# Lalwaniamisha789/Implementation-of-Neural-LDPC-Decoders-with-Degree-Specific-Weight-Sharing-and-RCQ-Quantization

Hardware: AMD Instinct MI355X
Metric: decoded codewords/sec at fixed iters; achieved HBM GB/s vs peak (higher is better)
Workload: dtype f32; 1 GPU; (1998,1512) IRA code, BasicMinSumDecoder factor=0.7, fp32, 10 iterations, batch 65536/GPU, SNR 2.0 dB, fixed-iteration flooding decode; graph=ira_1998_1512, n=1998, m=486, edges=6587, batch_per_gpu=65536, global_batch=65536, parallelism=dp1, collective=none

## Files before the change

### implementation-of-neural-ldpc-decoders-with-degree-specific-weight-sharing-and-rcq-quantization_amd/_native.py

```python

from __future__ import annotations

import ctypes as C
import os
import subprocess
import threading
from typing import Optional

import numpy as np

_HERE = os.path.dirname(os.path.abspath(__file__))
LIB_NAME = "libldpc_hip.so"
LIB_PATH = os.environ.get("LDPC_HIP_LIB") or os.path.join(_HERE, LIB_NAME)
CSRC = os.path.join(_HERE, "csrc")
HEADER = os.path.join(os.path.dirname(_HERE), "include", "ldpc_hip.h")
DEBUG_HEADER = os.path.join(os.path.dirname(_HERE), "include", "ldpc_hip_debug.h")

LDPC_F32, LDPC_F64 = 0, 1
C2V_NMS, C2V_RCQ, C2V_OMS = 0, 1, 2
MODE_AUTO, MODE_STREAM, MODE_RESIDENT, MODE_SWEEPS, MODE_GATHER, MODE_PAIR = 0, 1, 2, 3, 4, 5
SCHED_FLOODING, SCHED_LAYERED_REF, SCHED_LAYERED = 0, 1, 2

HIPCC_FLAGS = ["--offload-arch=gfx950", "-O3", "-std=c++17", "-fPIC", "-shared",
               "-ffp-contract=off",
# ... 67 lines not shown
                ("n_beta_slots", C.c_int32), ("beta", C.c_void_p), ("beta_slot", C.c_void_p),
                ("n_alpha_slots", C.c_int32), ("alpha", C.c_void_p), ("alpha_slot", C.c_void_p),
                ("n_levels", C.c_int32), ("n_quantizers", C.c_int32), ("thresholds", C.c_void_p),
                ("q_of_iter", C.c_void_p),
                ("n_oms_alpha_slots", C.c_int32), ("oms_alpha", C.c_void_p), ("oms_alpha_slot", C.c_void_p),
                ("schedule", C.c_int32)]


PRODUCT_EXPORTS = ("ldpc_graph_create", "ldpc_graph_destroy", "ldpc_graph_info", "ldpc_decoder_create",
                   "ldpc_decoder_set_mode", "ldpc_decoder_info",
                   "ldpc_decoder_set_weights", "ldpc_decoder_destroy", "ldpc_decoder_workspace_bytes",
                   "ldpc_decode", "ldpc_decode_capped", "ldpc_last_error", "ldpc_abi_version", "ldpc_source_hash",
                   "ldpc_train_saved_bytes", "ldpc_train_workspace_bytes", "ldpc_decode_saving", "ldpc_backward",
                   "ldpc_train_joint_workspace_bytes", "ldpc_train_joint")
DEBUG_EXPORTS = ("ldpc_debug_sweep", "ldpc_debug_workspace_layout", "ldpc_debug_resident_c2v", "ldpc_debug_key4",
                 "ldpc_debug_compact_layout", "ldpc_debug_compact_checks", "ldpc_debug_compact_banks")
EXPORTS = PRODUCT_EXPORTS + DEBUG_EXPORTS

_lib = None
_lock = threading.Lock()


def load():
    global _lib
    if _lib is not None:
        return _lib
    with _lock:
        if _lib is not None:
            return _lib
        if not os.path.exists(LIB_PATH):
            raise NativeEngineError(
# ... 32 lines not shown
        lib.ldpc_decode_capped.argtypes = [vp, vp, i64, i32, i32, vp, vp, vp, vp, vp, vp, C.c_size_t, vp]
        lib.ldpc_debug_sweep.restype = C.c_int
        lib.ldpc_debug_sweep.argtypes = [vp, i64, i32, i32, vp, C.c_size_t, vp]
        lib.ldpc_debug_workspace_layout.restype = C.c_int
        lib.ldpc_debug_workspace_layout.argtypes = [vp, i64, i32, vp]
        lib.ldpc_debug_key4.restype = C.c_int
        lib.ldpc_debug_key4.argtypes = [vp, i64, C.c_float, vp, vp, vp, vp]
        lib.ldpc_debug_resident_c2v.restype = C.c_int
        lib.ldpc_debug_resident_c2v.argtypes = [vp, vp, i64, i32, i32, vp, vp, vp, vp]
        lib.ldpc_debug_compact_layout.restype = C.c_int
        lib.ldpc_debug_compact_layout.argtypes = [vp, i32, i32, i32, vp, vp, vp, vp, vp]
        lib.ldpc_debug_compact_banks.restype = C.c_int
        lib.ldpc_debug_compact_banks.argtypes = [vp, i32, i32, i32, vp, vp, vp, vp, vp, vp, vp, vp, vp]
        lib.ldpc_debug_compact_checks.restype = C.c_int
        lib.ldpc_debug_compact_checks.argtypes = [vp, i32, i32, i32, vp, vp, vp]
        lib.ldpc_train_saved_bytes.restype = C.c_size_t
        lib.ldpc_train_saved_bytes.argtypes = [vp, i64]
        lib.ldpc_train_workspace_bytes.restype = C.c_size_t
        lib.ldpc_train_workspace_bytes.argtypes = [vp, i64]
        lib.ldpc_decode_saving.restype = C.c_int
        lib.ldpc_decode_saving.argtypes = [vp, vp, i64, i32, vp, vp, vp, vp, vp, C.c_size_t, vp, C.c_size_t, vp]
        lib.ldpc_backward.restype = C.c_int
        lib.ldpc_backward.argtypes = [vp, vp, C.c_size_t, vp, i64, vp, vp, vp, vp, vp, vp, vp, C.c_size_t, vp]
        lib.ldpc_train_joint_workspace_bytes.restype = C.c_size_t
        lib.ldpc_train_joint_workspace_bytes.argtypes = [vp, i64]
        lib.ldpc_train_joint.restype = C.c_int
        lib.ldpc_train_joint.argtypes = [vp, vp, vp, i64, vp, vp, vp, vp, vp, vp, vp, vp, vp, C.c_size_t, vp]
        lib.ldpc_last_error.restype = C.c_char_p
        lib.ldpc_last_error.argtypes = []
        lib.ldpc_abi_version.restype = C.c_int
# ... 22 lines not shown
```

### implementation-of-neural-ldpc-decoders-with-degree-specific-weight-sharing-and-rcq-quantization_amd/csrc/ldpc_hip.hip

```cpp
#include "ldpc_kernels.hip"
#include "ldpc_resident.hip"
#include "ldpc_train.hip"
#include "ldpc_layered.hip"

#include <algorithm>
#include <climits>
#include <mutex>
#include <set>
#include <cmath>
#include <cstdarg>
#include <cstdio>
#include <cstdlib>
#include <cstring>
#include <exception>
#include <new>
#include <vector>

#include "../../include/ldpc_hip.h"
#include "../../include/ldpc_hip_debug.h"

using namespace ldpc;

namespace {

// ... 1282 lines not shown

void cpt_layout(const ldpc_graph *g, const std::vector<ResVCheck> &vc, long long S, CptLayout &L)
{
    const int n = g->n;
    std::vector<int> dv(n);
    for (int j = 0; j < n; ++j) dv[j] = g->h_var_ptr[j + 1] - g->h_var_ptr[j];
    if (!cpt_assign(dv, L) || (long long)L.var_at.size() > S) {
        L.var_at.resize(n);
        for (int j = 0; j < n; ++j) L.var_at[j] = j;
        std::stable_sort(L.var_at.begin(), L.var_at.end(), [&](int a, int b) { return dv[a] > dv[b]; });
    }
    cpt_place_banks(g, vc, L);
    cpt_cells(dv, L);
}

int resident_layout(ldpc_decoder *d, const ldpc_decoder_desc *desc, const std::vector<ResVCheck> &sorted, int mstride,
                    long long S, int G, ResidentPlan &pl, const CptLayout *cl)
{
    const ldpc_graph *g = d->g;
    std::vector<ResVCheck> placed;
    if (cl)
        for (int c : cl->check_at) placed.push_back(sorted[c]);
    const std::vector<ResVCheck> &vc = cl ? placed : sorted;
    const int n = g->n, m = (int)vc.size();
    const bool any_split = m != g->m;
    int max_sub = 0;
    for (const ResVCheck &v : vc) max_sub = std::max(max_sub, v.dc);
    std::vector<int> perm_v(n), pos_v(n);
    for (int j = 0; j < n; ++j) perm_v[j] = j;
    auto dv_of = [&](int j) { return g->h_var_ptr[j + 1] - g->h_var_ptr[j]; };
    std::stable_sort(perm_v.begin(), perm_v.end(), [&](int a, int b) { return dv_of(a) > dv_of(b); });
    std::vector<int> slot_of_edge(g->E);
    for (int p = 0; p < m; ++p)
        for (int t = 0; t < vc[p].dc; ++t) slot_of_edge[vc[p].e0 + t] = t * mstride + p;
    if (cl) {
        perm_v = cl->var_at;
        slot_of_edge = cl->slot_of_edge;
    } else {
        std::vector<std::vector<int>> vs(n);
        for (int j = 0; j < n; ++j)
            for (int k = 0; k < dv_of(j); ++k) vs[j].push_back(slot_of_edge[g->h_csc[g->h_var_ptr[j] + k]]);
        optimise_lane_order(perm_v, vs, G);
    }
    const int n_pos = (int)perm_v.size();
    const int n_ent = cl ? (n_pos + 63) / 64 * 64 : n;
    for (int q = 0; q < n_pos; ++q)
        if (perm_v[q] >= 0) pos_v[perm_v[q]] = q;

    std::vector<uint8_t> dc_s(m), gsz(m);
    std::vector<uint16_t> cvar((size_t)S, 0), bslot((size_t)S, 0), oaslot((size_t)S, 0), bslot_c(m, 0), inv(n);
    std::vector<uint32_t> vmeta(n_ent, 0u);
    std::vector<uint2> vslot_lo(n_ent, make_uint2(0, kResHole)), vslot_hi(std::max(n_ent, 1), make_uint2(0, 0));
    int n_hi = 0;
    std::vector<uint32_t> edge_of_slot((size_t)S, 0xffffffffu);
    bool per_check = true;
    for (int p = 0; p < m; ++p) {
        const ResVCheck &v = vc[p];
        const int first = g->h_check_ptr[v.check];
        dc_s[p] = (uint8_t)v.dc;
        gsz[p] = (uint8_t)v.gs;
        for (int t = 0; t < v.dc; ++t) {
            const int e = v.e0 + t, slot = slot_of_edge[e];
            edge_of_slot[slot] = (uint32_t)e;
            cvar[slot] = (uint16_t)pos_v[g->h_var_idx[e]];
            bslot[slot] = (uint16_t)desc->beta_slot[e];
            if (desc->beta_slot[e] != desc->beta_slot[first]) per_check = false;
            if (d->form == LDPC_C2V_OMS && desc->oms_alpha) oaslot[slot] = (uint16_t)desc->oms_alpha_slot[e];
        }
        bslot_c[p] = v.dc ? (uint16_t)desc->beta_slot[first] : 0;
    }
    for (int q = 0; q < n_pos; ++q) {
        if (perm_v[q] < 0) continue;
        const int j = perm_v[q], s0 = g->h_var_ptr[j], dv = dv_of(j);
        vmeta[q] = (uint32_t)dv | ((uint32_t)desc->alpha_slot[j] << 8);
        inv[j] = (uint16_t)q;
        uint32_t off[8] = {0, 0, 0, 0, 0, 0, 0, 0};
        for (int k = 0; k < dv; ++k) off[k] = (uint32_t)slot_of_edge[g->h_csc[s0 + k]] * G * 4;
        vslot_lo[q] = make_uint2(off[0] | (off[1] << 16), off[2] | (off[3] << 16));
        vslot_hi[q] = make_uint2(off[4] | (off[5] << 16), off[6] | (off[7] << 16));
        if (dv > 4) n_hi = q + 1;
    }
    pl = ResidentPlan{};
    pl.n = n; pl.m = m; pl.S = (int)S; pl.max_dc = max_sub; pl.max_dv = g->max_dv; pl.mstride = mstride; pl.E = g->E;
    pl.any_split = any_split ? 1 : 0;
    pl.n_hi = n_hi;
    pl.n_pos = n_pos;
    if (cl) {
        std::copy(cl->cell, cl->cell + kCptWaves, pl.vcell);
        cpt_check_words(vc, per_check && (d->form == LDPC_C2V_NMS || (d->form == LDPC_C2V_RCQ && d->rcq_zero0)),
                        pl.ccell);
    }
    pl.par_words = is_pow2(mstride) ? m : 0;
    pl.par_shift = G == 2 ? 3 : 2;
    int rc = plan_upload(d, &pl.dc_s, dc_s);
    if (!rc && any_split) rc = plan_upload(d, &pl.gsz, gsz);
    if (!rc) rc = plan_upload(d, &pl.cvar, cvar);
    if (!rc) rc = plan_upload(d, &pl.bslot, bslot);
    if (!rc && per_check) rc = plan_upload(d, &pl.bslot_c, bslot_c);
    if (!rc && d->form == LDPC_C2V_OMS && desc->oms_alpha) rc = plan_upload(d, &pl.oaslot, oaslot);
    if (!rc) rc = plan_upload(d, &pl.vmeta, vmeta);
    if (!rc) rc = plan_upload(d, &pl.vslot_lo, vslot_lo);
    vslot_hi.resize((size_t)std::max(n_hi, 1));
    if (!rc) rc = plan_upload(d, &pl.vslot_hi, vslot_hi);
    if (!rc) rc = plan_upload(d, &pl.inv_perm_v, inv);
    if (!rc) rc = plan_upload(d, &pl.edge_of_slot, edge_of_slot);
    return rc;
}

int allow_full_lds(const void *kfn, int device)
{
    static std::mutex mu;
    static std::set<std::pair<const void *, int>> done;
    std::lock_guard<std::mutex> lk(mu);
    if (done.count({kfn, device})) return LDPC_OK;
    HIP_TRY(hipFuncSetAttribute(kfn, hipFuncAttributeMaxDynamicSharedMemorySize, (int)kLdsBytes));
    done.insert({kfn, device});
    return LDPC_OK;
// ... 1098 lines not shown
    emit(L->slot_of_edge, L->check_at, L->banks, slot_of_edge, pos_of_check, model);
    emit(L->base_slot_of_edge, L->base_check_at, L->base_banks, base_slot_of_edge, base_pos_of_check, base_model);
    if (geometry) { geometry[0] = kResCptStride; geometry[1] = (int32_t)Sc; }
    return LDPC_OK;
}

int ldpc_debug_compact_banks(const ldpc_decoder *d, int32_t n, int32_t m, int32_t E, const int32_t *check_ptr,
                             const int32_t *var_idx, int32_t *slot_of_edge, int32_t *pos_of_check, int32_t model[4],
                             int32_t *base_slot_of_edge, int32_t *base_pos_of_check, int32_t base_model[4],
                             int32_t geometry[2])
{
    LDPC_NOTHROW(compact_banks_impl(d, n, m, E, check_ptr, var_idx, slot_of_edge, pos_of_check, model, base_slot_of_edge,
                                    base_pos_of_check, base_model, geometry))
}

int ldpc_debug_resident_c2v(const ldpc_decoder *d, const void *llr, int64_t batch, int32_t early_stop,
                            int32_t max_iterations, void *posterior, int32_t *iterations, void *c2v_out, void *stream)
{
    if (!d || !llr || !posterior || !c2v_out || batch <= 0) return fail(LDPC_ERR_ARG, "bad argument");
    if (!use_resident(d)) return fail(LDPC_ERR_ARG, "the decoder is not on the LDS-resident engine");
    if (d->g->n == 0) return LDPC_OK;
    IterCap cap(max_iterations > 0 ? max_iterations : INT_MAX);
    return decode_resident(d, llr, batch, early_stop, nullptr, posterior, iterations, nullptr, nullptr, c2v_out, stream);
}

int ldpc_debug_sweep(const ldpc_decoder *d, int64_t batch, int32_t which, int32_t iter, void *workspace,
                     size_t workspace_bytes, void *stream)
{
    if (!d || !workspace || batch <= 0) return fail(LDPC_ERR_ARG, "bad argument");
    if (iter < 0 || iter >= d->T) return fail(LDPC_ERR_ARG, "iter outside [0, T)");
// ... 35 lines not shown
```

### implementation-of-neural-ldpc-decoders-with-degree-specific-weight-sharing-and-rcq-quantization_amd/csrc/ldpc_resident.hip

```cpp
#pragma once

#include "ldpc_kernels.hip"

namespace ldpc {

struct ResidentPlan {
    int n, m, S, max_dc, max_dv;
    int mstride;
    const uint8_t *dc_s;
    const uint8_t *gsz;
    int any_split;
    int par_words;
    int par_shift;
    const uint16_t *cvar;
    const uint16_t *bslot;
    const uint16_t *bslot_c;
    const uint16_t *oaslot;
    const uint32_t *vmeta;
    const uint2 *vslot_lo;
    const uint2 *vslot_hi;
    int n_hi;
    const uint16_t *inv_perm_v;
    int n_pos;
    unsigned vcell[8];
// ... 490 lines not shown
                const float r = d > 0.0f ? d : 0.0f;
                const float val = r - oa;
                o.x[g] = nonzero ? __uint_as_float(__float_as_uint(val) ^ sflip) : 0.0f;
            } else {
                const float w = __uint_as_float(__float_as_uint(b * raw) ^ sflip);
                const float rec = res_quant_rec<NL>(__builtin_fabsf(w), th, thr, n_levels);
                o.x[g] = flip_sign<float>(rec, (w < 0.0f) ? 1u : 0u);
            }
        }
        lds_store<P>(addr, o);
        slot += sstride;
    }
    }
}

template <int G, int FORM, bool BPC, int NL, int MS, typename T, bool SPLIT, bool CPT = false>
__device__ __forceinline__ void res_check_phase(const ResidentPlan &pl, unsigned char *smem,
                                                const T *__restrict__ beta_row,
                                                const T *__restrict__ oa_row,
                                                const float *__restrict__ thr, int n_levels, bool rcq_zero0,
                                                int dc_pre, T b_pre, int tid, int nt, unsigned cw = 0)
{
    float th[8];
    if (FORM == FORM_RCQ) {
#pragma unroll
        for (int q = 0; q < 8; ++q) th[q] = (q < n_levels) ? thr[q] : __builtin_nanf("");
    }
    if constexpr (CPT && BPC && (FORM == FORM_NMS || FORM == FORM_RCQ)) {
        static_assert(G == 2 && !SPLIT && std::is_same<T, float>::value, "compact: fp32 codeword pairs, whole checks");
        asm volatile("" : "+s"(cw));
// ... 37 lines not shown
    const unsigned off[8] = {slo.x, slo.y, slo.z, slo.w, shi.x, shi.y, shi.z, shi.w};
    P x[DV > 0 ? DV : 1];
#pragma unroll
    for (int k = 0; k < DV; ++k) x[k] = lds_load<P>(off[k]);
    P l = lreg ? *lreg : L[q];
    if constexpr (MODE == 0 || MODE == 2 || MODE == 4 || MODE == 6) {
        P out[DV > 0 ? DV : 1];
        auto v2c = [&](T llr, T sum) { return (MODE & 2) ? llr + sum : llr + a * sum; };
        unsigned byte = 0;
#pragma unroll
        for (int g = 0; g < G; ++g) {
            T xs[DV > 0 ? DV : 1];
#pragma unroll
            for (int k = 0; k < DV; ++k) xs[k] = x[k].x[g];
            if constexpr ((MODE & 4) != 0) byte |= ((l.x[g] + sum_ct<DV, -1, ORD, T>(xs)) < (T)0 ? 1u : 0u) << g;
            if constexpr (DV >= 1) out[0].x[g] = v2c(l.x[g], sum_ct<DV - 1, 0, ORD, T>(xs));
            if constexpr (DV >= 2) out[1].x[g] = v2c(l.x[g], sum_ct<DV - 1, 1, ORD, T>(xs));
            if constexpr (DV >= 3) out[2].x[g] = v2c(l.x[g], sum_ct<DV - 1, 2, ORD, T>(xs));
            if constexpr (DV >= 4) out[3].x[g] = v2c(l.x[g], sum_ct<DV - 1, 3, ORD, T>(xs));
            if constexpr (DV >= 5) out[4].x[g] = v2c(l.x[g], sum_ct<DV - 1, 4, ORD, T>(xs));
            if constexpr (DV >= 6) out[5].x[g] = v2c(l.x[g], sum_ct<DV - 1, 5, ORD, T>(xs));
            if constexpr (DV >= 7) out[6].x[g] = v2c(l.x[g], sum_ct<DV - 1, 6, ORD, T>(xs));
            if constexpr (DV >= 8) out[7].x[g] = v2c(l.x[g], sum_ct<DV - 1, 7, ORD, T>(xs));
        }
#pragma unroll
        for (int k = 0; k < DV; ++k) lds_store<P>(off[k], out[k]);
        if constexpr ((MODE & 4) != 0) {
            bits_s[q] = (uint8_t)byte;
            if (ps.par_off) {
#pragma unroll
                for (int k = 0; k < DV; ++k) lds_atomic_xor(ps.par_off + (((off[k] >> ps.shift) & ps.mask) << 2), byte);
// ... 21 lines not shown
                for (int k = 0; k < DV; ++k) lds_atomic_xor(ps.par_off + (((off[k] >> ps.shift) & ps.mask) << 2), byte);
            }
        }
        if (store) {
            if constexpr (MODE == 9) *lreg = l;
            else L[q] = l;
        }
    }
}

__device__ __forceinline__ uint4 plan_unpack(const uint2 &p)
{
    return make_uint4(p.x & 0xffffu, p.x >> 16, p.y & 0xffffu, p.y >> 16);
}

template <int G, int MODE, typename T, int DMAX = 8>
__device__ __forceinline__ void res_var_dispatch(unsigned char *smem, T *__restrict__ llr_s,
                                                 uint8_t *__restrict__ bits_s, int q, int dv, const uint4 &slo,
                                                 const uint4 &shi, T a, unsigned emask, const ParScatter &ps,
                                                 Pack<T, G> *lreg = nullptr)
{
#define LDPC_RV(D) \
    case D: if constexpr (D <= DMAX) res_var_body<G, D, MODE, T>(smem, llr_s, bits_s, q, slo, shi, a, emask, ps, lreg); break;
    switch (dv) {
        LDPC_RV(0) LDPC_RV(1) LDPC_RV(2) LDPC_RV(3) LDPC_RV(4) LDPC_RV(5) LDPC_RV(6) LDPC_RV(7) LDPC_RV(8)
    default: break;
    }
#undef LDPC_RV
}

constexpr int kResRegVars = 4;
template <typename T, int G>
struct ResVarState {
    unsigned meta[kResRegVars];
    uint2 plo[kResRegVars];
    uint2 phi0;
    Pack<T, G> l[kResRegVars];
    unsigned cells;
};

constexpr unsigned kCellEmpty = 0x00;
constexpr unsigned kCellHoles = 0x40;
constexpr unsigned kCellMixed = 0xff;
constexpr unsigned kResHole = 0xffffffffu;

template <int G, int MODE, typename T, int R>
__device__ __forceinline__ void res_var_round_cpt(const ResidentPlan &pl, unsigned char *smem, const T *__restrict__ alpha_glb,
                                                  unsigned emask, int tid, int nt, ResVarState<T, G> &st)
{
    constexpr int DMAX = R == 0 ? 8 : 4;
    const unsigned cd = (st.cells >> (8 * R)) & 0xffu;
    if (cd == kCellEmpty) return;
    const int q = tid + R * nt;
    const uint4 slo = plan_unpack(st.plo[R]), shi = R == 0 ? plan_unpack(st.phi0) : make_uint4(0, 0, 0, 0);
    T a = (T)0;
    if (MODE == 0) a = alpha_glb[pl.vmeta[q] >> 8];
    const ParScatter ps{};
    if (cd == kCellMixed) {
        res_var_dispatch<G, MODE, T, DMAX>(smem, nullptr, nullptr, q, (int)(pl.vmeta[q] & 0xffu), slo, shi, a, emask, ps,
                                           &st.l[R]);
        return;
    }
    if ((cd & kCellHoles) && st.plo[R].y == kResHole) return;
#define LDPC_RVU(D) \
    case D: if constexpr (D <= DMAX) res_var_body<G, D, MODE, T>(smem, nullptr, nullptr, q, slo, shi, a, emask, ps, &st.l[R]); break;
    switch (cd & 0xfu) {
        LDPC_RVU(1) LDPC_RVU(2) LDPC_RVU(3) LDPC_RVU(4) LDPC_RVU(5) LDPC_RVU(6) LDPC_RVU(7) LDPC_RVU(8)
    default: break;
    }
#undef LDPC_RVU
}

template <int G, int MODE, typename T>
__device__ __forceinline__ void res_var_phase_cpt(const ResidentPlan &pl, unsigned char *smem, const T *__restrict__ alpha_glb,
                                                  unsigned emask, int tid, int nt, ResVarState<T, G> &st)
{
#pragma unroll
    for (int r = 0; r < kResRegVars; ++r) asm volatile("" : "+v"(st.plo[r].x), "+v"(st.plo[r].y));
    asm volatile("" : "+v"(st.phi0.x), "+v"(st.phi0.y));
    static_assert(kResRegVars == 4, "four rounds");
    res_var_round_cpt<G, MODE, T, 0>(pl, smem, alpha_glb, emask, tid, nt, st);
    res_var_round_cpt<G, MODE, T, 1>(pl, smem, alpha_glb, emask, tid, nt, st);
    res_var_round_cpt<G, MODE, T, 2>(pl, smem, alpha_glb, emask, tid, nt, st);
    res_var_round_cpt<G, MODE, T, 3>(pl, smem, alpha_glb, emask, tid, nt, st);
}

template <int G, int MODE, typename T>
__device__ __forceinline__ void res_var_phase_reg(const ResidentPlan &pl, unsigned char *smem,
                                                  T *__restrict__ llr_s, uint8_t *__restrict__ bits_s,
                                                  const T *__restrict__ alpha_lds,
                                                  const T *__restrict__ alpha_glb, unsigned emask,
                                                  int tid, int nt, ResVarState<T, G> &st, const ParScatter &ps)
{
#pragma unroll
    for (int r = 0; r < kResRegVars; ++r) asm volatile("" : "+v"(st.meta[r]), "+v"(st.plo[r].x), "+v"(st.plo[r].y));
    asm volatile("" : "+v"(st.phi0.x), "+v"(st.phi0.y));
#pragma unroll
    for (int r = 0; r < kResRegVars; ++r) {
        const int q = tid + r * nt;
// ... 76 lines not shown

template <int G, bool SPLIT>
__device__ __forceinline__ void res_parity_reduce(const ResidentPlan &pl, unsigned par_off, unsigned *sh_unsat, int tid, int nt)
{
    unsigned acc = 0;
    for (int p = tid; p < pl.m; p += nt) {
        unsigned x = lds_load<unsigned>(par_off + 4u * (unsigned)p);
        lds_store<unsigned>(par_off + 4u * (unsigned)p, 0u);
        if constexpr (SPLIT) x = group_xor(pl.gsz[p], x);
        acc |= x;
    }
    if (acc) atomicOr(sh_unsat, acc);
}

template <int G, typename T, bool SPLIT>
__device__ __forceinline__ void res_syndrome_slots(const ResidentPlan &pl, unsigned *sh_unsat, int tid, int nt)
{
    constexpr unsigned kSlot = sizeof(Pack<T, G>);
    unsigned acc = 0;
    for (int p = tid; p < pl.m; p += nt) {
        const int dc = pl.dc_s[p];
        int dcw;
        unsigned x = 0;
        if (wave_uniform(dc, dcw)) {
#pragma unroll 8
            for (int t = 0; t < dcw; ++t) x ^= lds_load<unsigned>((unsigned)(t * pl.mstride + p) * kSlot);
        } else {
            for (int t = 0; t < dc; ++t) x ^= lds_load<unsigned>((unsigned)(t * pl.mstride + p) * kSlot);
        }
        if constexpr (SPLIT) x = group_xor(pl.gsz[p], x);
        acc |= x;
    }
    if (acc) atomicOr(sh_unsat, acc);
}

constexpr int kEmit = 4;

template <int G>
__device__ __forceinline__ void res_store_packed(const ResidentArgs &a, long long b, int j, int n, bool neg)
{
    const unsigned long long m = __ballot(neg);
    const int lane = threadIdx.x & 63;
    const int base = j - lane;
    if (lane < 8 && base + 8 * lane < n) a.packed[(size_t)b * ((n + 7) / 8) + (base >> 3) + lane] = (uint8_t)(m >> (8 * lane));
}

template <int G, typename T>
__device__ __forceinline__ void res_emit(const ResidentPlan &pl, const ResidentArgs &a, const T *__restrict__ llr_s,
                                         long long b0, unsigned mask, int iters, unsigned unsat, int tid, int nt)
{
    using P = Pack<T, G>;
    T *posterior = reinterpret_cast<T *>(a.posterior);
    const int n = pl.n;
    if (a.posterior || a.bits || a.packed) {
        for (int j0 = tid; j0 < n; j0 += kEmit * nt) {
            unsigned ip[kEmit];
#pragma unroll
            for (int k = 0; k < kEmit; ++k) ip[k] = (j0 + k * nt < n) ? pl.inv_perm_v[j0 + k * nt] : 0u;
#pragma unroll
            for (int k = 0; k < kEmit; ++k) {
                const int j = j0 + k * nt;
                if (j - (tid & 63) >= n) break;
                const bool in = j < n;
                const P p = reinterpret_cast<const P *>(llr_s)[ip[k]];
#pragma unroll
                for (int g = 0; g < G; ++g) {
                    if (!((mask >> g) & 1u)) continue;
                    if (in && a.posterior) res_stream_store(&posterior[(size_t)(b0 + g) * n + j], p.x[g]);
                    if (in && a.bits) res_stream_store(&a.bits[(size_t)(b0 + g) * n + j], p.x[g] < (T)0 ? 1 : 0);
                    if (a.packed) res_store_packed<G>(a, b0 + g, j, n, in && p.x[g] < (T)0);
                }
            }
        }
// ... 60 lines not shown
    }
}

__host__ __device__ inline size_t res_off_llr(int S, int G) { return (size_t)S * G * 4; }
__host__ __device__ inline size_t res_off_alpha(int S, int n, int G) { return res_off_llr(S, G) + (size_t)n * G * 4; }
__host__ __device__ inline size_t res_off_bits(int S, int n, int G, int n_alpha_lds) { return res_off_alpha(S, n, G) + (size_t)n_alpha_lds * 4; }
__host__ __device__ inline size_t res_off_flag(int S, int n, int G, int n_alpha_lds) { return (res_off_bits(S, n, G, n_alpha_lds) + n + 3) / 4 * 4; }
__host__ __device__ inline size_t res_off_par(int S, int n, int G, int n_alpha_lds) { return res_off_flag(S, n, G, n_alpha_lds) + 16; }
__host__ __device__ inline size_t res_lds_total(int S, int n, int G, int n_alpha_lds, int m_par) { return res_off_par(S, n, G, n_alpha_lds) + 4 * (size_t)m_par; }

__host__ __device__ inline size_t res_cpt_off_flag(int S, int G) { return ((size_t)S * G * 4 + 15) / 16 * 16; }
__host__ __device__ inline size_t res_cpt_lds_total(int S, int G) { return res_cpt_off_flag(S, G) + 16; }

constexpr int kResMaxThreads = 1024;
constexpr int kResMinWaves = 4;
constexpr int kResCptThreads = 512;
constexpr int kResCptWaves = 6;
constexpr int kResCptBlocks = 3;
constexpr int kResCptStride = 495;
template <int G, int FORM, bool BPC, int NL, int MS, int ES, typename T = float, bool SPLIT = false, bool REG = false,
          bool CPT = false>
__global__ __launch_bounds__(CPT ? kResCptThreads : kResMaxThreads, CPT ? kResCptWaves : kResMinWaves)
void resident_decode(ResidentPlan pl, ResidentArgs a)
{
    static_assert(!CPT || (REG && !ES && !SPLIT && std::is_same<T, float>::value), "compact: fixed-T fp32 REG kernels only");
    extern __shared__ __align__(16) unsigned char res_smem[];
    if (__builtin_amdgcn_groupstaticsize() != 0) __builtin_trap();
    constexpr int GE = G * (int)(sizeof(T) / 4);
    const int n_alpha_lds = a.alpha_in_lds ? a.T * a.n_alpha * (int)(sizeof(T) / 4) : 0;
    T *llr_s = reinterpret_cast<T *>(res_smem + (CPT ? 0 : res_off_llr(pl.S, GE)));
    T *alpha_s = reinterpret_cast<T *>(res_smem + res_off_alpha(pl.S, pl.n, GE));
    uint8_t *bits_s = res_smem + res_off_bits(pl.S, pl.n, GE, n_alpha_lds);
    unsigned *sh_unsat = reinterpret_cast<unsigned *>(res_smem + (CPT ? res_cpt_off_flag(pl.S, GE)
// ... 2 lines not shown
    if (pl.par_words) {
        psf.par_off = (unsigned)res_off_par(pl.S, pl.n, GE, n_alpha_lds);
        psf.shift = (unsigned)pl.par_shift;
        psf.mask = (unsigned)pl.mstride - 1u;
        if (ES) ps = psf;
    }
    const T *g_llr = reinterpret_cast<const T *>(a.llr);
    const T *g_beta = reinterpret_cast<const T *>(a.beta);
    const T *g_alpha = reinterpret_cast<const T *>(a.alpha);
    const T *g_oms_alpha = reinterpret_cast<const T *>(a.oms_alpha);
    using P = Pack<T, G>;
    const int tid = threadIdx.x, nt = blockDim.x, n = pl.n;
    const long long b0 = (long long)blockIdx.x * G;
    constexpr unsigned kAll = (1u << G) - 1u;

    constexpr int kPro = 4;
    for (int j0 = tid; j0 < n; j0 += kPro * nt) {
        unsigned ip[kPro];
        P v[kPro];
#pragma unroll
        for (int k = 0; k < kPro; ++k) {
            const int j = j0 + k * nt;
            ip[k] = 0;
            if (j < n) {
                ip[k] = pl.inv_perm_v[j];
#pragma unroll
                for (int g = 0; g < G; ++g)
                    v[k].x[g] = (b0 + g < a.batch) ? res_stream_load(&g_llr[(size_t)(b0 + g) * n + j]) : (T)1;
            }
        }
#pragma unroll
        for (int k = 0; k < kPro; ++k)
            if (j0 + k * nt < n) reinterpret_cast<P *>(llr_s)[ip[k]] = v[k];
    }
    for (int k = tid; k < (a.alpha_in_lds ? a.T * a.n_alpha : 0); k += nt) alpha_s[k] = g_alpha[k];
    if (tid == 0) { sh_unsat[0] = 0; sh_unsat[1] = 0; }
    for (int k = tid; k < pl.par_words; k += nt) lds_store<unsigned>(psf.par_off + 4u * (unsigned)k, 0u);
    __syncthreads();
    ResVarState<T, G> st{};
    if constexpr (CPT) {
        st.cells = pl.vcell[__builtin_amdgcn_readfirstlane(tid) >> 6];
        const P *L = reinterpret_cast<const P *>(llr_s);
#pragma unroll
        for (int r = 0; r < kResRegVars; ++r) {
            const int q = tid + r * nt;
            if (q < pl.n_pos) st.l[r] = L[q];
            if ((st.cells >> (8 * r)) & 0xffu) {
                st.plo[r] = pl.vslot_lo[q];
                if (r == 0 && q < pl.n_hi) st.phi0 = pl.vslot_hi[q];
            }
        }
        __syncthreads();
#pragma unroll
        for (int r = 0; r < kResRegVars; ++r) {
            const unsigned cd = (st.cells >> (8 * r)) & 0xffu;
            if (cd == kCellEmpty) continue;
            const int q = tid + r * nt;
            int dv = (int)(cd & 0xfu);
            if (cd == kCellMixed) dv = (int)(pl.vmeta[q] & 0xffu);
            else if ((cd & kCellHoles) && st.plo[r].y == kResHole) dv = 0;
            const uint4 slo = plan_unpack(st.plo[r]), shi = r == 0 ? plan_unpack(st.phi0) : make_uint4(0, 0, 0, 0);
            const unsigned off[8] = {slo.x, slo.y, slo.z, slo.w, shi.x, shi.y, shi.z, shi.w};
            P l = st.l[r];
            if (a.T == 0) {
#pragma unroll
                for (int g = 0; g < G; ++g) l.x[g] = (T)0;
            }
#pragma unroll
            for (int e = 0; e < (r == 0 ? 8 : 4); ++e)
                if (e < dv) lds_store<P>(off[e], l);
        }
    } else if constexpr (REG) {
        const P *L = reinterpret_cast<const P *>(llr_s);
#pragma unroll
        for (int r = 0; r < kResRegVars; ++r) {
            const int q = tid + r * nt;
// ... 51 lines not shown
                    if constexpr (!std::is_same<T, float>::value) {
#pragma unroll
                        for (int g = 0; g < G; ++g) l.x[g] = __builtin_canonicalize(l.x[g]);
                    }
                    if (a.T == 0) {
#pragma unroll
                        for (int g = 0; g < G; ++g) l.x[g] = (T)0;
                    }
#pragma unroll
                    for (int e = 0; e < 8; ++e)
                        if (e < dvk[k]) lds_store<P>(off[e], l);
                }
            }
        }
    }
    unsigned chk_cells = 0;
    if constexpr (CPT) chk_cells = pl.ccell[__builtin_amdgcn_readfirstlane(tid) >> 6];
    const int dc_pre = tid < pl.m ? pl.dc_s[tid] : 0;
    T b_pre = (BPC && tid < pl.m && a.T > 0) ? g_beta[pl.bslot_c[tid]] : (T)0;
    __syncthreads();

    unsigned done = 0;
#pragma unroll
    for (int g = 0; g < G; ++g)
        if (b0 + g >= a.batch) done |= 1u << g;

    for (int it = 0; it < a.T; ++it) {
        const T *beta_row = g_beta + (size_t)it * a.n_beta;
        const T *oa_row = a.oms_alpha ? g_oms_alpha + (size_t)it * a.n_oms_alpha : nullptr;
        const float *thr = FORM == FORM_RCQ ? a.thr + (size_t)a.q_of_iter[it] * a.n_levels : nullptr;
        const T *alpha_lds = a.alpha_in_lds ? alpha_s + it * a.n_alpha : nullptr;
        const T *alpha_glb = g_alpha + (size_t)it * a.n_alpha;
        res_check_phase<G, FORM, BPC, NL, MS, T, SPLIT, CPT>(pl, res_smem, beta_row, oa_row, thr, a.n_levels,
                                                             a.rcq_zero0 != 0, dc_pre, b_pre, tid, nt, chk_cells);
        if (BPC && tid < pl.m && it + 1 < a.T)
            b_pre = g_beta[(size_t)(it + 1) * a.n_beta + pl.bslot_c[tid]];
        __syncthreads();
        if (ES && !a.posterior) {
            const bool last = it == a.T - 1;
            if (last) res_var_phase<G, 1, T, REG>(pl, res_smem, llr_s, bits_s, (const T *)nullptr, (const T *)nullptr, 0u, tid, nt, st, ps);
            else if (a.unit_alpha) res_var_phase<G, 6, T, REG>(pl, res_smem, llr_s, bits_s, (const T *)nullptr, (const T *)nullptr, 0u, tid, nt, st, ps);
            else res_var_phase<G, 4, T, REG>(pl, res_smem, llr_s, bits_s, alpha_lds, alpha_glb, 0u, tid, nt, st, ps);
            __syncthreads();
            unsigned *su = sh_unsat + (it & 1);
            if (ps.par_off) res_parity_reduce<G, SPLIT>(pl, ps.par_off, su, tid, nt);
            else res_syndrome_phase<G, SPLIT>(pl, bits_s, su, tid, nt);
            __syncthreads();
            const unsigned unsat = *su;
            if (tid == 0) sh_unsat[(it + 1) & 1] = 0;
            const unsigned newly = ~unsat & ~done & kAll;
            if (newly) {
// ... 37 lines not shown
        unsigned real = 0;
#pragma unroll
        for (int g = 0; g < G; ++g)
            if (b0 + g < a.batch) real |= 1u << g;
        res_dump_c2v<G, T>(pl, a, b0, open & real, tid, nt);
        __syncthreads();
    }
    if (ES && !a.posterior && a.T > 0) {
        res_emit_bits<G>(pl, a, bits_s, b0, open, a.T, kAll, tid, nt);
        return;
    }
    const bool scatter = !ES && !CPT && psf.par_off != 0;
    if (ES) res_var_phase<G, 1, T, REG>(pl, res_smem, llr_s, bits_s, (const T *)nullptr, (const T *)nullptr, open, tid, nt, st);
    else if (scatter) res_var_phase<G, 1, T, REG>(pl, res_smem, llr_s, bits_s, (const T *)nullptr, (const T *)nullptr, open, tid, nt, st, psf);
    else res_var_phase<G, CPT ? 9 : 8, T, REG, CPT>(pl, res_smem, llr_s, bits_s, (const T *)nullptr, (const T *)nullptr, open, tid, nt, st);
    __syncthreads();
    unsigned unsat = kAll;
    if (!ES) {
        if (scatter) res_parity_reduce<G, SPLIT>(pl, psf.par_off, sh_unsat, tid, nt);
        else res_syndrome_slots<G, T, SPLIT>(pl, sh_unsat, tid, nt);
        __syncthreads();
        unsat = *sh_unsat;
    }
    if constexpr (CPT) {
#pragma unroll
        for (int r = 0; r < kResRegVars; ++r)
            if (tid + r * nt < pl.n_pos) reinterpret_cast<P *>(llr_s)[tid + r * nt] = st.l[r];
        __syncthreads();
    }
    res_emit<G, T>(pl, a, llr_s, b0, open, a.T, unsat, tid, nt);
}

}
```

### include/ldpc_hip_debug.h

```cpp
#ifndef LDPC_HIP_DEBUG_H
#define LDPC_HIP_DEBUG_H

#include "ldpc_hip.h"

#ifdef __cplusplus
extern "C" {
#endif

int ldpc_debug_sweep(const ldpc_decoder *d, int64_t batch, int32_t which, int32_t iter,
                     void *workspace, size_t workspace_bytes, void *stream);

int ldpc_debug_workspace_layout(const ldpc_decoder *d, int64_t batch, int32_t max_iterations, int64_t out8[8]);

int ldpc_debug_resident_c2v(const ldpc_decoder *d, const void *llr, int64_t batch, int32_t early_stop,
                            int32_t max_iterations, void *posterior, int32_t *iterations, void *c2v_out,
                            void *stream);

int ldpc_debug_compact_layout(const ldpc_decoder *d, int32_t n, int32_t m, int32_t E, const int32_t *check_ptr,
                              const int32_t *var_idx, int32_t *pos_of_var, uint8_t cells[32], int32_t stats[4]);

int ldpc_debug_compact_checks(const ldpc_decoder *d, int32_t n, int32_t m, int32_t E, const int32_t *check_ptr,
                              const int32_t *var_idx, uint32_t words[8]);

int ldpc_debug_compact_banks(const ldpc_decoder *d, int32_t n, int32_t m, int32_t E, const int32_t *check_ptr,
                             const int32_t *var_idx, int32_t *slot_of_edge, int32_t *pos_of_check, int32_t model[4],
                             int32_t *base_slot_of_edge, int32_t *base_pos_of_check, int32_t base_model[4],
                             int32_t geometry[2]);

int ldpc_debug_key4(const float *values, int64_t count, float beta, const float thresholds4[4], uint8_t *keys_float,
                    uint8_t *keys_compare, void *stream);

#ifdef __cplusplus
}
#endif
#endif
```

Baseline: 35.35 million codewords/s.

## Hoist compact-plan loads into kernel prologue and pack degree into slot words

For the compact resident (CPT) kernel, the per-thread plan words (vslot_lo/hi, cell masks, check degree and beta column) are now loaded unconditionally at kernel start, before the LLR prologue, from padded fixed-size tables. The variable degree is packed into the low bits of the slot offsets, so the mixed-cell path no longer reads vmeta. Alpha values for all four rounds are fetched together, and the emit-stage inverse permutation is prefetched before the final barrier. The goal is to take dependent global loads off the critical path and overlap them with other work. In exchange the plan tables are padded and use more registers, and a debug export is added to inspect the plan.

```diff
diff --git a/implementation-of-neural-ldpc-decoders-with-degree-specific-weight-sharing-and-rcq-quantization_amd/_native.py b/implementation-of-neural-ldpc-decoders-with-degree-specific-weight-sharing-and-rcq-quantization_amd/_native.py
--- a/implementation-of-neural-ldpc-decoders-with-degree-specific-weight-sharing-and-rcq-quantization_amd/_native.py
+++ b/implementation-of-neural-ldpc-decoders-with-degree-specific-weight-sharing-and-rcq-quantization_amd/_native.py
@@ -105,7 +105,8 @@
                    "ldpc_train_saved_bytes", "ldpc_train_workspace_bytes", "ldpc_decode_saving", "ldpc_backward",
                    "ldpc_train_joint_workspace_bytes", "ldpc_train_joint")
 DEBUG_EXPORTS = ("ldpc_debug_sweep", "ldpc_debug_workspace_layout", "ldpc_debug_resident_c2v", "ldpc_debug_key4",
-                 "ldpc_debug_compact_layout", "ldpc_debug_compact_checks", "ldpc_debug_compact_banks")
+                 "ldpc_debug_compact_layout", "ldpc_debug_compact_checks", "ldpc_debug_compact_banks",
+                 "ldpc_debug_compact_plan")
 EXPORTS = PRODUCT_EXPORTS + DEBUG_EXPORTS
 
 _lib = None
@@ -168,6 +169,8 @@
         lib.ldpc_debug_compact_banks.argtypes = [vp, i32, i32, i32, vp, vp, vp, vp, vp, vp, vp, vp, vp]
         lib.ldpc_debug_compact_checks.restype = C.c_int
         lib.ldpc_debug_compact_checks.argtypes = [vp, i32, i32, i32, vp, vp, vp]
+        lib.ldpc_debug_compact_plan.restype = C.c_int
+        lib.ldpc_debug_compact_plan.argtypes = [vp, i32, i32, i32, vp, vp, vp, vp, vp, vp]
         lib.ldpc_train_saved_bytes.restype = C.c_size_t
         lib.ldpc_train_saved_bytes.argtypes = [vp, i64]
         lib.ldpc_train_workspace_bytes.restype = C.c_size_t
diff --git a/implementation-of-neural-ldpc-decoders-with-degree-specific-weight-sharing-and-rcq-quantization_amd/csrc/ldpc_hip.hip b/implementation-of-neural-ldpc-decoders-with-degree-specific-weight-sharing-and-rcq-quantization_amd/csrc/ldpc_hip.hip
--- a/implementation-of-neural-ldpc-decoders-with-degree-specific-weight-sharing-and-rcq-quantization_amd/csrc/ldpc_hip.hip
+++ b/implementation-of-neural-ldpc-decoders-with-degree-specific-weight-sharing-and-rcq-quantization_amd/csrc/ldpc_hip.hip
@@ -1320,6 +1320,19 @@
     cpt_cells(dv, L);
 }
 
+void plan_entry(const ldpc_graph *g, const std::vector<int> &slot_of_edge, int j, int G, bool compact, uint2 &lo, uint2 &hi)
+{
+    const int s0 = g->h_var_ptr[j], dv = g->h_var_ptr[j + 1] - s0;
+    uint32_t off[8] = {0, 0, 0, 0, 0, 0, 0, 0};
+    for (int k = 0; k < dv; ++k) off[k] = (uint32_t)slot_of_edge[g->h_csc[s0 + k]] * G * 4;
+    lo = make_uint2(off[0] | (off[1] << 16), off[2] | (off[3] << 16));
+    if (compact) {
+        const unsigned l4[4] = {off[0], off[1], off[2], off[3]};
+        lo = plan_pack_cpt(l4, (unsigned)dv);
+    }
+    hi = make_uint2(off[4] | (off[5] << 16), off[6] | (off[7] << 16));
+}
+
 int resident_layout(ldpc_decoder *d, const ldpc_decoder_desc *desc, const std::vector<ResVCheck> &sorted, int mstride,
                     long long S, int G, ResidentPlan &pl, const CptLayout *cl)
 {
@@ -1349,12 +1362,13 @@
         optimise_lane_order(perm_v, vs, G);
     }
     const int n_pos = (int)perm_v.size();
-    const int n_ent = cl ? (n_pos + 63) / 64 * 64 : n;
+    const int n_ent = cl ? kResRegVars * kResCptThreads : n;
+    const int m_ent = cl ? kResCptThreads : m;
     for (int q = 0; q < n_pos; ++q)
         if (perm_v[q] >= 0) pos_v[perm_v[q]] = q;
 
-    std::vector<uint8_t> dc_s(m), gsz(m);
-    std::vector<uint16_t> cvar((size_t)S, 0), bslot((size_t)S, 0), oaslot((size_t)S, 0), bslot_c(m, 0), inv(n);
+    std::vector<uint8_t> dc_s(m_ent, 0), gsz(m);
+    std::vector<uint16_t> cvar((size_t)S, 0), bslot((size_t)S, 0), oaslot((size_t)S, 0), bslot_c(m_ent, 0), inv(n);
     std::vector<uint32_t> vmeta(n_ent, 0u);
     std::vector<uint2> vslot_lo(n_ent, make_uint2(0, kResHole)), vslot_hi(std::max(n_ent, 1), make_uint2(0, 0));
     int n_hi = 0;
@@ -1377,13 +1391,10 @@
     }
     for (int q = 0; q < n_pos; ++q) {
         if (perm_v[q] < 0) continue;
-        const int j = perm_v[q], s0 = g->h_var_ptr[j], dv = dv_of(j);
+        const int j = perm_v[q], dv = dv_of(j);
         vmeta[q] = (uint32_t)dv | ((uint32_t)desc->alpha_slot[j] << 8);
         inv[j] = (uint16_t)q;
-        uint32_t off[8] = {0, 0, 0, 0, 0, 0, 0, 0};
-        for (int k = 0; k < dv; ++k) off[k] = (uint32_t)slot_of_edge[g->h_csc[s0 + k]] * G * 4;
-        vslot_lo[q] = make_uint2(off[0] | (off[1] << 16), off[2] | (off[3] << 16));
-        vslot_hi[q] = make_uint2(off[4] | (off[5] << 16), off[6] | (off[7] << 16));
+        plan_entry(g, slot_of_edge, j, G, cl != nullptr, vslot_lo[q], vslot_hi[q]);
         if (dv > 4) n_hi = q + 1;
     }
     pl = ResidentPlan{};
@@ -1406,7 +1417,7 @@
     if (!rc && d->form == LDPC_C2V_OMS && desc->oms_alpha) rc = plan_upload(d, &pl.oaslot, oaslot);
     if (!rc) rc = plan_upload(d, &pl.vmeta, vmeta);
     if (!rc) rc = plan_upload(d, &pl.vslot_lo, vslot_lo);
-    vslot_hi.resize((size_t)std::max(n_hi, 1));
+    vslot_hi.resize((size_t)(cl ? kResCptThreads : std::max(n_hi, 1)));
     if (!rc) rc = plan_upload(d, &pl.vslot_hi, vslot_hi);
     if (!rc) rc = plan_upload(d, &pl.inv_perm_v, inv);
     if (!rc) rc = plan_upload(d, &pl.edge_of_slot, edge_of_slot);
@@ -2535,6 +2546,49 @@
                                     base_pos_of_check, base_model, geometry))
 }
 
+static int compact_plan_impl(const ldpc_decoder *d, int32_t n, int32_t m, int32_t E, const int32_t *check_ptr,
+                             const int32_t *var_idx, uint32_t *vslot_lo, uint32_t *vslot_hi, uint32_t *vcell, uint32_t *ccell)
+{
+    CptLayout own;
+    ldpc_graph own_g;
+    const CptLayout *L = &own;
+    const ldpc_graph *g = &own_g;
+    unsigned words[kCptWaves];
+    if (d) {
+        if (!d->resc_ok) return fail(LDPC_ERR_UNSUPPORTED, "the decoder has no compact fixed-T plan");
+        L = &d->resc_layout;
+        g = d->g;
+        std::copy(d->resc.ccell, d->resc.ccell + kCptWaves, words);
+    } else {
+        if (int rc = graph_host_build(&own_g, n, m, E, check_ptr, var_idx)) return rc;
+        std::vector<ResVCheck> vc;
+        long long Sc = 0;
+        if (!resident_checks(g, vc) || !cpt_geometry(g, vc, Sc))
+            return fail(LDPC_ERR_UNSUPPORTED, "the graph does not qualify for the compact plan");
+        cpt_layout(g, vc, Sc, own);
+        std::vector<ResVCheck> placed;
+        for (int c : own.check_at) placed.push_back(vc[c]);
+        cpt_check_words(placed, true, words);
+    }
+    constexpr int kPos = kResRegVars * kResCptThreads;
+    for (int q = 0; q < kPos; ++q) {
+        uint2 lo = make_uint2(0, kResHole), hi = make_uint2(0, 0);
+        if (q < (int)L->var_at.size() && L->var_at[q] >= 0) plan_entry(g, L->slot_of_edge, L->var_at[q], 2, true, lo, hi);
+        if (vslot_lo) { vslot_lo[2 * q] = lo.x; vslot_lo[2 * q + 1] = lo.y; }
+        if (vslot_hi && q < kResCptThreads) { vslot_hi[2 * q] = hi.x; vslot_hi[2 * q + 1] = hi.y; }
+    }
+    if (vcell) std::copy(L->cell, L->cell + kCptWaves, vcell);
+    if (ccell) std::copy(words, words + kCptWaves, ccell);
+    return LDPC_OK;
+}
+
+int ldpc_debug_compact_plan(const ldpc_decoder *d, int32_t n, int32_t m, int32_t E, const int32_t *check_ptr,
+                            const int32_t *var_idx, uint32_t *vslot_lo, uint32_t *vslot_hi, uint32_t vcell[8],
+                            uint32_t ccell[8])
+{
+    LDPC_NOTHROW(compact_plan_impl(d, n, m, E, check_ptr, var_idx, vslot_lo, vslot_hi, vcell, ccell))
+}
+
 int ldpc_debug_resident_c2v(const ldpc_decoder *d, const void *llr, int64_t batch, int32_t early_stop,
                             int32_t max_iterations, void *posterior, int32_t *iterations, void *c2v_out, void *stream)
 {
diff --git a/implementation-of-neural-ldpc-decoders-with-degree-specific-weight-sharing-and-rcq-quantization_amd/csrc/ldpc_resident.hip b/implementation-of-neural-ldpc-decoders-with-degree-specific-weight-sharing-and-rcq-quantization_amd/csrc/ldpc_resident.hip
--- a/implementation-of-neural-ldpc-decoders-with-degree-specific-weight-sharing-and-rcq-quantization_amd/csrc/ldpc_resident.hip
+++ b/implementation-of-neural-ldpc-decoders-with-degree-specific-weight-sharing-and-rcq-quantization_amd/csrc/ldpc_resident.hip
@@ -528,6 +528,15 @@
     }
 }
 
+template <typename T>
+__device__ __forceinline__ unsigned res_chk_word(unsigned dc, unsigned col) { return dc | (col * (unsigned)sizeof(T)) << 8; }
+__device__ __forceinline__ int res_chk_dc(unsigned w) { return (int)(w & 0xffu); }
+template <typename T>
+__device__ __forceinline__ T res_beta_at(const T *__restrict__ row, unsigned w)
+{
+    return *reinterpret_cast<const T *>(reinterpret_cast<const char *>(row) + (size_t)(w >> 8));
+}
+
 template <int G, int FORM, bool BPC, int NL, int MS, typename T, bool SPLIT, bool CPT = false>
 __device__ __forceinline__ void res_check_phase(const ResidentPlan &pl, unsigned char *smem,
                                                 const T *__restrict__ beta_row,
@@ -595,7 +604,12 @@
 #pragma unroll
             for (int k = 0; k < DV; ++k) xs[k] = x[k].x[g];
             if constexpr ((MODE & 4) != 0) byte |= ((l.x[g] + sum_ct<DV, -1, ORD, T>(xs)) < (T)0 ? 1u : 0u) << g;
-            if constexpr (DV >= 1) out[0].x[g] = v2c(l.x[g], sum_ct<DV - 1, 0, ORD, T>(xs));
+            if constexpr (DV == 1) {
+                T z = sum_ct<0, 0, ORD, T>(xs);
+                asm volatile("" : "+v"(z));
+                out[0].x[g] = v2c(l.x[g], z);
+            }
+            if constexpr (DV >= 2) out[0].x[g] = v2c(l.x[g], sum_ct<DV - 1, 0, ORD, T>(xs));
             if constexpr (DV >= 2) out[1].x[g] = v2c(l.x[g], sum_ct<DV - 1, 1, ORD, T>(xs));
             if constexpr (DV >= 3) out[2].x[g] = v2c(l.x[g], sum_ct<DV - 1, 2, ORD, T>(xs));
             if constexpr (DV >= 4) out[3].x[g] = v2c(l.x[g], sum_ct<DV - 1, 3, ORD, T>(xs));
@@ -647,6 +661,17 @@
     return make_uint4(p.x & 0xffffu, p.x >> 16, p.y & 0xffffu, p.y >> 16);
 }
 
+constexpr unsigned kResHole = 0xfffffffeu;
+__host__ __device__ inline uint2 plan_pack_cpt(const unsigned (&off)[4], unsigned dv)
+{
+    return make_uint2((off[0] | (dv & 7u)) | (off[1] << 16), (off[2] | (dv >> 3)) | (off[3] << 16));
+}
+__host__ __device__ inline uint4 plan_unpack_cpt(const uint2 &p)
+{
+    return make_uint4(p.x & 0xfff8u, p.x >> 16, p.y & 0xfff8u, p.y >> 16);
+}
+__host__ __device__ inline unsigned plan_degree_cpt(const uint2 &p) { return (p.x & 7u) | (p.y & 1u) << 3; }
+
 template <int G, int MODE, typename T, int DMAX = 8>
 __device__ __forceinline__ void res_var_dispatch(unsigned char *smem, T *__restrict__ llr_s,
                                                  uint8_t *__restrict__ bits_s, int q, int dv, const uint4 &slo,
@@ -663,6 +688,9 @@
 }
 
 constexpr int kResRegVars = 4;
+constexpr int kResCptThreads = 512;
+constexpr int kResCptWaves = 6;
+constexpr int kResCptBlocks = 3;
 template <typename T, int G>
 struct ResVarState {
     unsigned meta[kResRegVars];
@@ -675,22 +703,19 @@
 constexpr unsigned kCellEmpty = 0x00;
 constexpr unsigned kCellHoles = 0x40;
 constexpr unsigned kCellMixed = 0xff;
-constexpr unsigned kResHole = 0xffffffffu;
 
 template <int G, int MODE, typename T, int R>
-__device__ __forceinline__ void res_var_round_cpt(const ResidentPlan &pl, unsigned char *smem, const T *__restrict__ alpha_glb,
-                                                  unsigned emask, int tid, int nt, ResVarState<T, G> &st)
+__device__ __forceinline__ void res_var_round_cpt(unsigned char *smem, T a, unsigned emask, int tid, int nt,
+                                                  ResVarState<T, G> &st)
 {
     constexpr int DMAX = R == 0 ? 8 : 4;
     const unsigned cd = (st.cells >> (8 * R)) & 0xffu;
     if (cd == kCellEmpty) return;
     const int q = tid + R * nt;
-    const uint4 slo = plan_unpack(st.plo[R]), shi = R == 0 ? plan_unpack(st.phi0) : make_uint4(0, 0, 0, 0);
-    T a = (T)0;
-    if (MODE == 0) a = alpha_glb[pl.vmeta[q] >> 8];
+    const uint4 slo = plan_unpack_cpt(st.plo[R]), shi = R == 0 ? plan_unpack(st.phi0) : make_uint4(0, 0, 0, 0);
     const ParScatter ps{};
     if (cd == kCellMixed) {
-        res_var_dispatch<G, MODE, T, DMAX>(smem, nullptr, nullptr, q, (int)(pl.vmeta[q] & 0xffu), slo, shi, a, emask, ps,
+        res_var_dispatch<G, MODE, T, DMAX>(smem, nullptr, nullptr, q, (int)plan_degree_cpt(st.plo[R]), slo, shi, a, emask, ps,
                                            &st.l[R]);
         return;
     }
@@ -712,10 +737,24 @@
     for (int r = 0; r < kResRegVars; ++r) asm volatile("" : "+v"(st.plo[r].x), "+v"(st.plo[r].y));
     asm volatile("" : "+v"(st.phi0.x), "+v"(st.phi0.y));
     static_assert(kResRegVars == 4, "four rounds");
-    res_var_round_cpt<G, MODE, T, 0>(pl, smem, alpha_glb, emask, tid, nt, st);
-    res_var_round_cpt<G, MODE, T, 1>(pl, smem, alpha_glb, emask, tid, nt, st);
-    res_var_round_cpt<G, MODE, T, 2>(pl, smem, alpha_glb, emask, tid, nt, st);
-    res_var_round_cpt<G, MODE, T, 3>(pl, smem, alpha_glb, emask, tid, nt, st);
+    T a[kResRegVars] = {};
+    if constexpr (MODE == 0) {
+        unsigned meta[kResRegVars] = {};
+        unsigned o = (unsigned)tid << 2;
+        asm volatile("" : "+v"(o));
+#pragma unroll
+        for (int r = 0; r < kResRegVars; ++r)
+            meta[r] = *reinterpret_cast<const uint32_t *>(reinterpret_cast<const char *>(pl.vmeta) +
+                                                              (size_t)(o + (unsigned)(r * kResCptThreads * 4)));
+#pragma unroll
+        for (int r = 0; r < kResRegVars; ++r)
+            a[r] = *reinterpret_cast<const T *>(reinterpret_cast<const char *>(alpha_glb) +
+                                                    (size_t)((meta[r] >> 8) * (unsigned)sizeof(T)));
+    }
+    res_var_round_cpt<G, MODE, T, 0>(smem, a[0], emask, tid, nt, st);
+    res_var_round_cpt<G, MODE, T, 1>(smem, a[1], emask, tid, nt, st);
+    res_var_round_cpt<G, MODE, T, 2>(smem, a[2], emask, tid, nt, st);
+    res_var_round_cpt<G, MODE, T, 3>(smem, a[3], emask, tid, nt, st);
 }
 
 template <int G, int MODE, typename T>
@@ -822,12 +861,12 @@
 }
 
 template <int G, typename T, bool SPLIT>
-__device__ __forceinline__ void res_syndrome_slots(const ResidentPlan &pl, unsigned *sh_unsat, int tid, int nt)
+__device__ __forceinline__ void res_syndrome_slots(const ResidentPlan &pl, unsigned *sh_unsat, int tid, int nt, int dc_own = -1)
 {
     constexpr unsigned kSlot = sizeof(Pack<T, G>);
     unsigned acc = 0;
     for (int p = tid; p < pl.m; p += nt) {
-        const int dc = pl.dc_s[p];
+        const int dc = dc_own >= 0 ? dc_own : (int)pl.dc_s[p];
         int dcw;
         unsigned x = 0;
         if (wave_uniform(dc, dcw)) {
@@ -853,9 +892,18 @@
     if (lane < 8 && base + 8 * lane < n) a.packed[(size_t)b * ((n + 7) / 8) + (base >> 3) + lane] = (uint8_t)(m >> (8 * lane));
 }
 
+__device__ __forceinline__ void res_emit_fetch(const ResidentPlan &pl, int j0, int nt, unsigned (&ip)[kEmit])
+{
+#pragma unroll
+    for (int k = 0; k < kEmit; ++k)
+        ip[k] = (j0 + k * nt < pl.n) ? *reinterpret_cast<const uint16_t *>(reinterpret_cast<const char *>(pl.inv_perm_v) +
+                                                                            (size_t)((unsigned)(j0 + k * nt) << 1)) : 0u;
+}
+
 template <int G, typename T>
 __device__ __forceinline__ void res_emit(const ResidentPlan &pl, const ResidentArgs &a, const T *__restrict__ llr_s,
-                                         long long b0, unsigned mask, int iters, unsigned unsat, int tid, int nt)
+                                         long long b0, unsigned mask, int iters, unsigned unsat, int tid, int nt,
+                                         const unsigned (*ip_first)[kEmit] = nullptr)
 {
     using P = Pack<T, G>;
     T *posterior = reinterpret_cast<T *>(a.posterior);
@@ -863,8 +911,12 @@
     if (a.posterior || a.bits || a.packed) {
         for (int j0 = tid; j0 < n; j0 += kEmit * nt) {
             unsigned ip[kEmit];
-#pragma unroll
-            for (int k = 0; k < kEmit; ++k) ip[k] = (j0 + k * nt < n) ? pl.inv_perm_v[j0 + k * nt] : 0u;
+            if (ip_first && j0 == tid) {
+#pragma unroll
+                for (int k = 0; k < kEmit; ++k) ip[k] = (*ip_first)[k];
+            } else {
+                res_emit_fetch(pl, j0, nt, ip);
+            }
 #pragma unroll
             for (int k = 0; k < kEmit; ++k) {
                 const int j = j0 + k * nt;
@@ -955,9 +1007,6 @@
 
 constexpr int kResMaxThreads = 1024;
 constexpr int kResMinWaves = 4;
-constexpr int kResCptThreads = 512;
-constexpr int kResCptWaves = 6;
-constexpr int kResCptBlocks = 3;
 constexpr int kResCptStride = 495;
 template <int G, int FORM, bool BPC, int NL, int MS, int ES, typename T = float, bool SPLIT = false, bool REG = false,
           bool CPT = false>
@@ -990,6 +1039,22 @@
     const long long b0 = (long long)blockIdx.x * G;
     constexpr unsigned kAll = (1u << G) - 1u;
 
+    ResVarState<T, G> st{};
+    unsigned chk_cells = 0;
+    unsigned chk_pre = 0;
+    unsigned dc_raw = 0, col_raw = 0;
+    if constexpr (CPT) {
+        const int wave = __builtin_amdgcn_readfirstlane(tid) >> 6;
+        st.cells = pl.vcell[wave];
+        chk_cells = pl.ccell[wave];
+#pragma unroll
+        for (int r = 0; r < kResRegVars; ++r)
+            st.plo[r] = *reinterpret_cast<const uint2 *>(reinterpret_cast<const char *>(pl.vslot_lo) +
+                                                         (size_t)((unsigned)(tid + r * kResCptThreads) << 3));
+        st.phi0 = *reinterpret_cast<const uint2 *>(reinterpret_cast<const char *>(pl.vslot_hi) + (size_t)((unsigned)tid << 3));
+        dc_raw = *(reinterpret_cast<const uint8_t *>(pl.dc_s) + (size_t)(unsigned)tid);
+        if (BPC) col_raw = *reinterpret_cast<const uint16_t *>(reinterpret_cast<const char *>(pl.bslot_c) + (size_t)((unsigned)tid << 1));
+    }
     constexpr int kPro = 4;
     for (int j0 = tid; j0 < n; j0 += kPro * nt) {
         unsigned ip[kPro];
@@ -1009,33 +1074,31 @@
         for (int k = 0; k < kPro; ++k)
             if (j0 + k * nt < n) reinterpret_cast<P *>(llr_s)[ip[k]] = v[k];
     }
-    for (int k = tid; k < (a.alpha_in_lds ? a.T * a.n_alpha : 0); k += nt) alpha_s[k] = g_alpha[k];
+    if constexpr (!CPT)
+        for (int k = tid; k < (a.alpha_in_lds ? a.T * a.n_alpha : 0); k += nt) alpha_s[k] = g_alpha[k];
     if (tid == 0) { sh_unsat[0] = 0; sh_unsat[1] = 0; }
-    for (int k = tid; k < pl.par_words; k += nt) lds_store<unsigned>(psf.par_off + 4u * (unsigned)k, 0u);
+    if constexpr (!CPT)
+        for (int k = tid; k < pl.par_words; k += nt) lds_store<unsigned>(psf.par_off + 4u * (unsigned)k, 0u);
+    T b_pre = (T)0;
+    if constexpr (CPT) {
+        chk_pre = res_chk_word<T>(dc_raw, col_raw);
+        b_pre = (BPC && a.T > 0) ? res_beta_at<T>(g_beta, chk_pre) : (T)0;
+    }
     __syncthreads();
-    ResVarState<T, G> st{};
     if constexpr (CPT) {
-        st.cells = pl.vcell[__builtin_amdgcn_readfirstlane(tid) >> 6];
         const P *L = reinterpret_cast<const P *>(llr_s);
 #pragma unroll
-        for (int r = 0; r < kResRegVars; ++r) {
-            const int q = tid + r * nt;
-            if (q < pl.n_pos) st.l[r] = L[q];
-            if ((st.cells >> (8 * r)) & 0xffu) {
-                st.plo[r] = pl.vslot_lo[q];
-                if (r == 0 && q < pl.n_hi) st.phi0 = pl.vslot_hi[q];
-            }
-        }
+        for (int r = 0; r < kResRegVars; ++r)
+            if (tid + r * nt < pl.n_pos) st.l[r] = L[tid + r * nt];
         __syncthreads();
 #pragma unroll
         for (int r = 0; r < kResRegVars; ++r) {
             const unsigned cd = (st.cells >> (8 * r)) & 0xffu;
             if (cd == kCellEmpty) continue;
-            const int q = tid + r * nt;
             int dv = (int)(cd & 0xfu);
-            if (cd == kCellMixed) dv = (int)(pl.vmeta[q] & 0xffu);
+            if (cd == kCellMixed) dv = (int)plan_degree_cpt(st.plo[r]);
             else if ((cd & kCellHoles) && st.plo[r].y == kResHole) dv = 0;
-            const uint4 slo = plan_unpack(st.plo[r]), shi = r == 0 ? plan_unpack(st.phi0) : make_uint4(0, 0, 0, 0);
+            const uint4 slo = plan_unpack_cpt(st.plo[r]), shi = r == 0 ? plan_unpack(st.phi0) : make_uint4(0, 0, 0, 0);
             const unsigned off[8] = {slo.x, slo.y, slo.z, slo.w, shi.x, shi.y, shi.z, shi.w};
             P l = st.l[r];
             if (a.T == 0) {
@@ -1117,10 +1180,10 @@
             }
         }
     }
-    unsigned chk_cells = 0;
-    if constexpr (CPT) chk_cells = pl.ccell[__builtin_amdgcn_readfirstlane(tid) >> 6];
-    const int dc_pre = tid < pl.m ? pl.dc_s[tid] : 0;
-    T b_pre = (BPC && tid < pl.m && a.T > 0) ? g_beta[pl.bslot_c[tid]] : (T)0;
+    if constexpr (!CPT) {
+        if (tid < pl.m) chk_pre = res_chk_word<T>(pl.dc_s[tid], BPC ? pl.bslot_c[tid] : 0u);
+        b_pre = (BPC && a.T > 0) ? res_beta_at<T>(g_beta, chk_pre) : (T)0;
+    }
     __syncthreads();
 
     unsigned done = 0;
@@ -1134,10 +1197,11 @@
         const float *thr = FORM == FORM_RCQ ? a.thr + (size_t)a.q_of_iter[it] * a.n_levels : nullptr;
         const T *alpha_lds = a.alpha_in_lds ? alpha_s + it * a.n_alpha : nullptr;
         const T *alpha_glb = g_alpha + (size_t)it * a.n_alpha;
+        asm volatile("" : "+v"(chk_pre));
         res_check_phase<G, FORM, BPC, NL, MS, T, SPLIT, CPT>(pl, res_smem, beta_row, oa_row, thr, a.n_levels,
-                                                             a.rcq_zero0 != 0, dc_pre, b_pre, tid, nt, chk_cells);
-        if (BPC && tid < pl.m && it + 1 < a.T)
-            b_pre = g_beta[(size_t)(it + 1) * a.n_beta + pl.bslot_c[tid]];
+                                                             a.rcq_zero0 != 0, res_chk_dc(chk_pre), b_pre, tid, nt, chk_cells);
+        if (BPC && it + 1 < a.T)
+            b_pre = res_beta_at<T>(g_beta + (size_t)(it + 1) * a.n_beta, chk_pre);
         __syncthreads();
         if (ES && !a.posterior) {
             const bool last = it == a.T - 1;
@@ -1205,11 +1269,13 @@
     if (ES) res_var_phase<G, 1, T, REG>(pl, res_smem, llr_s, bits_s, (const T *)nullptr, (const T *)nullptr, open, tid, nt, st);
     else if (scatter) res_var_phase<G, 1, T, REG>(pl, res_smem, llr_s, bits_s, (const T *)nullptr, (const T *)nullptr, open, tid, nt, st, psf);
     else res_var_phase<G, CPT ? 9 : 8, T, REG, CPT>(pl, res_smem, llr_s, bits_s, (const T *)nullptr, (const T *)nullptr, open, tid, nt, st);
+    unsigned ip_first[kEmit] = {};
+    if constexpr (CPT) res_emit_fetch(pl, tid, nt, ip_first);
     __syncthreads();
     unsigned unsat = kAll;
     if (!ES) {
         if (scatter) res_parity_reduce<G, SPLIT>(pl, psf.par_off, sh_unsat, tid, nt);
-        else res_syndrome_slots<G, T, SPLIT>(pl, sh_unsat, tid, nt);
+        else res_syndrome_slots<G, T, SPLIT>(pl, sh_unsat, tid, nt, CPT ? res_chk_dc(chk_pre) : -1);
         __syncthreads();
         unsat = *sh_unsat;
     }
@@ -1219,7 +1285,7 @@
             if (tid + r * nt < pl.n_pos) reinterpret_cast<P *>(llr_s)[tid + r * nt] = st.l[r];
         __syncthreads();
     }
-    res_emit<G, T>(pl, a, llr_s, b0, open, a.T, unsat, tid, nt);
-}
-
-}
+    res_emit<G, T>(pl, a, llr_s, b0, open, a.T, unsat, tid, nt, CPT ? &ip_first : nullptr);
+}
+
+}
diff --git a/include/ldpc_hip_debug.h b/include/ldpc_hip_debug.h
--- a/include/ldpc_hip_debug.h
+++ b/include/ldpc_hip_debug.h
@@ -27,6 +27,10 @@
                              int32_t *base_slot_of_edge, int32_t *base_pos_of_check, int32_t base_model[4],
                              int32_t geometry[2]);
 
+int ldpc_debug_compact_plan(const ldpc_decoder *d, int32_t n, int32_t m, int32_t E, const int32_t *check_ptr,
+                            const int32_t *var_idx, uint32_t *vslot_lo, uint32_t *vslot_hi, uint32_t vcell[8],
+                            uint32_t ccell[8]);
+
 int ldpc_debug_key4(const float *values, int64_t count, float beta, const float thresholds4[4], uint8_t *keys_float,
                     uint8_t *keys_compare, void *stream);
 
```

Measured after the change: 35.73 million codewords/s (median of 4 runs). 1.01x the previous value.
